# facebookresearch/actionmesh

Hardware: NVIDIA H100
Metric: denoiser_steps_per_sec (higher is better)
Workload: dtype bf16

## Files before the change

### actionmesh_b200/csrc/gemm.cu

```cuda
#include <atomic>
#include <cstdlib>
#include "common.cuh"
#include "ptx.cuh"
#include "../../include/actionmesh_b200.h"

namespace amb {

constexpr int BM = 128;
constexpr int BK = 64;
constexpr int GEMM_THREADS = 384;
constexpr int CLUSTER = 2;
constexpr int GROUP_M = 8;
constexpr int EPI_BATCH = 4;

struct GemmParams {
  int M, N, K;
  int k_split_blocks;
  void* C;
  long long ldc;
  int c_fp32;
  const float* bias;
  const void* residual;
  long long ldr;
  int res_fp32;
  int act;
  const float* col_scale;
  int grp_rows, grp_stride, row_off;
  int norm_cols, norm_seg;
  const float* norm_w0;
  const float* norm_w1;
  float norm_eps;
  int rope_cols;
  const float* rope_cos;
  const float* rope_sin;
  int rope_rows_per_pos;
  void* C2;
  long long ldc2;
};

__device__ __forceinline__ float gelu_erf(float x) {
  const float ax = fabsf(x);
  float t;
  asm("rcp.approx.ftz.f32 %0, %1;" : "=f"(t) : "f"(fmaf(0.3275911f * 0.70710678118654752440f, ax, 1.0f)));
  float p = fmaf(t, 1.061405429f, -1.453152027f);
  p = fmaf(p, t, 1.421413741f);
  p = fmaf(p, t, -0.284496736f);
  p = fmaf(p, t, 0.254829592f);
  const float e = ex2_approx(ax * ax * (-0.5f * 1.4426950408889634f));
  const float q = 0.5f * (p * t) * e;
  return x * (x >= 0.0f ? 1.0f - q : q);
}

template <int BN>
struct GemmSmem {
  static constexpr int STAGES = BN == 128 ? 6 : 8;
  static constexpr int A_BYTES = BM * BK * 2;
  static constexpr int B_BYTES = BN * BK * 2;
  static constexpr int STAGE_BYTES = A_BYTES + B_BYTES;
  static constexpr int BAR_OFFSET = STAGES * STAGE_BYTES;
  static constexpr int TOTAL = BAR_OFFSET + 2 * STAGES * 8 + 1024;
};

__device__ __forceinline__ void store2(void* C, int c_fp32, long long off, float v0, float v1) {
  if (c_fp32) *reinterpret_cast<float2*>(reinterpret_cast<float*>(C) + off) = make_float2(v0, v1);
  else *reinterpret_cast<uint32_t*>(reinterpret_cast<__nv_bfloat16*>(C) + off) = pack_bf16(v0, v1);
}
__device__ __forceinline__ float2 load2(const void* R, int r_fp32, long long off) {
  if (r_fp32) return *reinterpret_cast<const float2*>(reinterpret_cast<const float*>(R) + off);
  return unpack_bf16(*reinterpret_cast<const uint32_t*>(reinterpret_cast<const __nv_bfloat16*>(R) + off));
}

__device__ __forceinline__ void finish_pair(const GemmParams& p, float v0, float v1, float2 r, long long drow, int col,
                                            bool valid) {
  if (p.bias) {
    const float2 b = __ldg(reinterpret_cast<const float2*>(p.bias + col));
    v0 += b.x; v1 += b.y;
  }
  if (p.act == 1) {
    v0 = gelu_erf(v0);
    v1 = gelu_erf(v1);
  }
  if (p.col_scale) {
    const float2 s = __ldg(reinterpret_cast<const float2*>(p.col_scale + col));
    v0 *= s.x; v1 *= s.y;
  }
  if (!valid) return;
  if (p.residual) { v0 += r.x; v1 += r.y; }
  store2(p.C, p.c_fp32, drow * p.ldc + col, v0, v1);
  if (p.C2) store2(p.C2, 0, drow * p.ldc2 + col, v0, v1);
}

template <int BN>
__device__ __forceinline__ void epilogue_tile(const GemmParams& p, const float* acc, int n0, int r0) {
  const int q = threadIdx.x & 3;
  long long drow[2];
  bool valid[2];
  int row[2] = {r0, r0 + 8};
#pragma unroll
  for (int h = 0; h < 2; ++h) {
    valid[h] = row[h] < p.M;
    drow[h] = row[h];
    if (p.grp_rows > 0) drow[h] = (long long)(row[h] / p.grp_rows) * p.grp_stride + (row[h] % p.grp_rows) + p.row_off;
  }
  if constexpr (BN == 128) {
    const bool do_norm = n0 < p.norm_cols, do_rope = n0 < p.rope_cols;
    if (do_norm || do_rope) {
      float rs[2] = {1.0f, 1.0f};
      float2 nw[16];
      if (do_norm) {
        const float* w = (n0 < p.norm_seg) ? p.norm_w0 : p.norm_w1;
#pragma unroll
        for (int i = 0; i < 16; ++i) nw[i] = __ldg(reinterpret_cast<const float2*>(w + 8 * i + 2 * q));
        float ss0 = 0.f, ss1 = 0.f;
#pragma unroll
        for (int i = 0; i < 16; ++i) {
          ss0 += acc[4 * i] * acc[4 * i] + acc[4 * i + 1] * acc[4 * i + 1];
          ss1 += acc[4 * i + 2] * acc[4 * i + 2] + acc[4 * i + 3] * acc[4 * i + 3];
        }
        ss0 += __shfl_xor_sync(0xffffffffu, ss0, 1);
        ss1 += __shfl_xor_sync(0xffffffffu, ss1, 1);
        ss0 += __shfl_xor_sync(0xffffffffu, ss0, 2);
        ss1 += __shfl_xor_sync(0xffffffffu, ss1, 2);
        rs[0] = rsqrtf(ss0 * (1.0f / 128.0f) + p.norm_eps);
        rs[1] = rsqrtf(ss1 * (1.0f / 128.0f) + p.norm_eps);
      }
#pragma unroll
      for (int h = 0; h < 2; ++h) {
        float rc[16], rsn[16];
        if (do_rope) {
          const int pos = (valid[h] ? row[h] : 0) / p.rope_rows_per_pos;
          const float* cs = p.rope_cos + (long long)pos * 64;
          const float* sn = p.rope_sin + (long long)pos * 64;
#pragma unroll
          for (int i = 0; i < 16; ++i) {
            rc[i] = __ldg(cs + 4 * i + q);
            rsn[i] = __ldg(sn + 4 * i + q);
          }
        }
#pragma unroll
        for (int i = 0; i < 16; ++i) {
          const int lc = 8 * i + 2 * q;
          float v0 = acc[4 * i + 2 * h], v1 = acc[4 * i + 2 * h + 1];
          if (do_norm) {
            v0 *= rs[h] * nw[i].x;
            v1 *= rs[h] * nw[i].y;
          }
          if (do_rope) {
            const float c = rc[i], s = rsn[i];
            const float x = v0, y = v1;
            v0 = x * c - y * s;
            v1 = y * c + x * s;
          }
          if (valid[h]) store2(p.C, p.c_fp32, drow[h] * p.ldc + n0 + lc, v0, v1);
        }
      }
      return;
    }
  }
#pragma unroll
  for (int i0 = 0; i0 < BN / 8; i0 += EPI_BATCH) {
    float2 r[EPI_BATCH][2];
#pragma unroll
    for (int i = 0; i < EPI_BATCH; ++i)
#pragma unroll
      for (int h = 0; h < 2; ++h)
        r[i][h] = (p.residual && valid[h]) ? load2(p.residual, p.res_fp32, drow[h] * p.ldr + n0 + 8 * (i0 + i) + 2 * q)
                                           : make_float2(0.f, 0.f);
#pragma unroll
    for (int i = 0; i < EPI_BATCH; ++i) {
      const int col = n0 + 8 * (i0 + i) + 2 * q;
      const float* a = acc + 4 * (i0 + i);
      finish_pair(p, a[0], a[1], r[i][0], drow[0], col, valid[0]);
      finish_pair(p, a[2], a[3], r[i][1], drow[1], col, valid[1]);
    }
  }
}

template <int BN>
__device__ __forceinline__ void wgmma_tile_k16(float* acc, uint64_t adesc, uint64_t bdesc) {
  if constexpr (BN == 128) wgmma_ss_n128(acc, adesc, bdesc, 1u);
  else wgmma_ss_n64(acc, adesc, bdesc, 1u);
}

__device__ __forceinline__ void unit_tile(int u, int num_mp, int num_n, uint32_t rank, int& m0, int& nt) {
  const int band = u / (GROUP_M * num_n);
  const int first = band * GROUP_M;
  const int rows = min(GROUP_M, num_mp - first);
  const int r = u - band * GROUP_M * num_n;
  m0 = ((first + r % rows) * CLUSTER + (int)rank) * BM;
  nt = r / rows;
}

template <int BN>
__global__ void __cluster_dims__(CLUSTER, 1, 1) __launch_bounds__(GEMM_THREADS, 1)
gemm_bf16_kernel(const __grid_constant__ CUtensorMap tmA, const __grid_constant__ CUtensorMap tmA2,
                 const __grid_constant__ CUtensorMap tmB, const GemmParams p) {
  using L = GemmSmem<BN>;
  constexpr int STAGES = L::STAGES;
  constexpr int B_HALF = L::B_BYTES / CLUSTER;
  extern __shared__ uint8_t smem_raw[];
  uint8_t* smem = reinterpret_cast<uint8_t*>((reinterpret_cast<uintptr_t>(smem_raw) + 1023) & ~uintptr_t(1023));
  uint64_t* full_bar = reinterpret_cast<uint64_t*>(smem + L::BAR_OFFSET);
  uint64_t* empty_bar = full_bar + STAGES;

  const int wg = __shfl_sync(0xffffffffu, threadIdx.x >> 7, 0);
  const int warp = threadIdx.x >> 5;
  const int lane = threadIdx.x & 31;
  const uint32_t rank = cluster_ctarank();
  if (threadIdx.x == 0) {
    tma_prefetch_desc(&tmA);
    tma_prefetch_desc(&tmA2);
    tma_prefetch_desc(&tmB);
    for (int s = 0; s < STAGES; ++s) {
      mbar_init(&full_bar[s], 1);
      mbar_init(&empty_bar[s], 4 * CLUSTER);
    }
    fence_mbar_init();
  }
  cluster_sync();

  const int num_n = p.N / BN;
  const int num_mp = (p.M + CLUSTER * BM - 1) / (CLUSTER * BM);
  const int num_units = num_mp * num_n;
  const int cluster = blockIdx.x / CLUSTER, num_clusters = gridDim.x / CLUSTER;
  const int num_kb = p.K / BK;

  if (wg == 0) {
    reg_dealloc<40>();
    if (warp == 0) {
      int s = 0;
      uint32_t phase = 0;
      for (int u = cluster; u < num_units; u += num_clusters) {
        int m0, nt;
        unit_tile(u, num_mp, num_n, rank, m0, nt);
        const int n0 = nt * BN;
        for (int kb = 0; kb < num_kb; ++kb) {
          mbar_wait(&empty_bar[s], phase ^ 1);
          if (elect_one()) {
            mbar_expect_tx(&full_bar[s], L::STAGE_BYTES);
            uint8_t* sa = smem + s * L::STAGE_BYTES;
            uint8_t* sb = sa + L::A_BYTES;
            if (kb < p.k_split_blocks) tma_load_2d(sa, &tmA, &full_bar[s], kb * BK, m0, kEvictNormal);
            else tma_load_2d(sa, &tmA2, &full_bar[s], (kb - p.k_split_blocks) * BK, m0, kEvictNormal);
            tma_load_2d_multicast(sb + rank * B_HALF, &tmB, &full_bar[s], kb * BK, n0 + (int)rank * (BN / CLUSTER),
                                  (uint16_t)((1u << CLUSTER) - 1), kEvictLast);
          }
          __syncwarp();
          if (++s == STAGES) { s = 0; phase ^= 1; }
        }
      }
      for (int j = 0; j < STAGES; ++j) {
        mbar_wait(&empty_bar[s], phase ^ 1);
        if (++s == STAGES) { s = 0; phase ^= 1; }
      }
    }
  } else {
    reg_alloc<232>();
    const uint32_t my_turn = wg, other_turn = 3 - wg;
    const int n_local = (num_units - cluster + num_clusters - 1) / num_clusters;
    for (int i = wg - 1; i < n_local; i += 2) {
      int m0, nt;
      unit_tile(cluster + i * num_clusters, num_mp, num_n, rank, m0, nt);
      const int n0 = nt * BN;
      float acc[2][BN / 2];
#pragma unroll
      for (int h = 0; h < 2; ++h)
#pragma unroll
        for (int j = 0; j < BN / 2; ++j) acc[h][j] = 0.f;
      const long long g0 = (long long)i * num_kb;
      int s = (int)(g0 % STAGES), s_prev = s;
      uint32_t phase = (uint32_t)((g0 / STAGES) & 1);
      if (i > 0) named_bar_sync(my_turn, 256);
      for (int kb = 0; kb < num_kb; ++kb) {
        mbar_wait_watched(&full_bar[s], phase);
        const uint32_t a_addr = smem_u32(smem + s * L::STAGE_BYTES);
        const uint64_t adesc0 = make_desc_kmajor_sw128(a_addr);
        const uint64_t adesc1 = make_desc_kmajor_sw128(a_addr + 64 * 128);
        const uint64_t bdesc = make_desc_kmajor_sw128(a_addr + L::A_BYTES);
        wgmma_fence();
#pragma unroll
        for (int k = 0; k < BK / 16; ++k) {
          wgmma_tile_k16<BN>(acc[0], adesc0 + 2 * k, bdesc + 2 * k);
          wgmma_tile_k16<BN>(acc[1], adesc1 + 2 * k, bdesc + 2 * k);
        }
        wgmma_commit();
        wgmma_wait<1>();
        if (kb > 0) {
          __syncwarp();
          if (lane < CLUSTER) mbar_arrive_cluster(&empty_bar[s_prev], lane);
        }
        s_prev = s;
        if (++s == STAGES) { s = 0; phase ^= 1; }
      }
      if (i + 1 < n_local) named_bar_arrive(other_turn, 256);
      wgmma_wait<0>();
#pragma unroll
      for (int h = 0; h < 2; ++h)
#pragma unroll
        for (int j = 0; j < BN / 2; ++j) reg_fence(acc[h][j]);
      __syncwarp();
      if (lane < CLUSTER) mbar_arrive_cluster(&empty_bar[s_prev], lane);
      if (m0 < p.M) {
        const int r0 = m0 + (warp & 3) * 16 + (lane >> 2);
        epilogue_tile<BN>(p, acc[0], n0, r0);
        epilogue_tile<BN>(p, acc[1], n0, r0 + 64);
      }
    }
  }
  __syncwarp();
  cluster_sync();
}

static GemmParams make_params(const amb_gemm_args* a) {
  GemmParams p;
  p.M = a->m; p.N = a->n; p.K = a->k;
  p.k_split_blocks = a->a2 ? a->k_split / BK : 0x7fffffff;
  p.C = a->c; p.ldc = a->ldc; p.c_fp32 = a->c_fp32;
  p.bias = a->bias;
  p.residual = a->residual; p.ldr = a->ldr; p.res_fp32 = a->res_fp32;
  p.act = a->act;
  p.col_scale = a->col_scale;
  p.grp_rows = a->grp_rows; p.grp_stride = a->grp_stride; p.row_off = a->row_off;
  p.norm_cols = a->norm_cols; p.norm_seg = a->norm_seg;
  p.norm_w0 = a->norm_w0; p.norm_w1 = a->norm_w1 ? a->norm_w1 : a->norm_w0;
  p.norm_eps = a->norm_eps;
  p.rope_cols = a->rope_cols; p.rope_cos = a->rope_cos; p.rope_sin = a->rope_sin;
  p.rope_rows_per_pos = a->rope_rows_per_pos > 0 ? a->rope_rows_per_pos : 1;
  p.C2 = a->c2; p.ldc2 = a->ldc2;
  return p;
}

template <int BN>
static int max_active_clusters(int* out) {
  static std::atomic<int> cached[16];
  int dev = 0;
  AMB_CHECK_CUDA(cudaGetDevice(&dev));
  if (dev < 16 && cached[dev].load() > 0) {
    *out = cached[dev].load();
    return AMB_OK;
  }
  cudaLaunchConfig_t cfg = {};
  cfg.gridDim = dim3(CLUSTER * num_sms(), 1, 1);
  cfg.blockDim = dim3(GEMM_THREADS, 1, 1);
  cfg.dynamicSmemBytes = GemmSmem<BN>::TOTAL;
  int n = 0;
  AMB_CHECK_CUDA(cudaOccupancyMaxActiveClusters(&n, gemm_bf16_kernel<BN>, &cfg));
  AMB_CHECK_ARG(n > 0, "gemm: no %d-CTA cluster of %d B shared memory fits on device %d", CLUSTER, GemmSmem<BN>::TOTAL, dev);
  if (dev < 16) cached[dev].store(n);
  *out = n;
  return AMB_OK;
}

template <int BN>
static int launch_gemm(const amb_gemm_args* a, cudaStream_t stream) {
  using L = GemmSmem<BN>;
  CUtensorMap tmA, tmA2, tmB;
  const int k1 = (a->a2 != nullptr) ? a->k_split : a->k;
  {
    uint64_t dims[2] = {(uint64_t)k1, (uint64_t)a->m};
    uint64_t str[1] = {(uint64_t)a->lda * 2};
    uint32_t box[2] = {BK, BM};
    int r = encode_tmap_bf16(&tmA, a->a, 2, dims, str, box);
    if (r) return r;
  }
  if (a->a2) {
    uint64_t dims[2] = {(uint64_t)(a->k - a->k_split), (uint64_t)a->m};
    uint64_t str[1] = {(uint64_t)a->lda2 * 2};
    uint32_t box[2] = {BK, BM};
    int r = encode_tmap_bf16(&tmA2, a->a2, 2, dims, str, box);
    if (r) return r;
  } else {
    tmA2 = tmA;
  }
  {
    uint64_t dims[2] = {(uint64_t)a->k, (uint64_t)a->n};
    uint64_t str[1] = {(uint64_t)a->ldw * 2};
    uint32_t box[2] = {BK, BN / CLUSTER};
    int r = encode_tmap_bf16(&tmB, a->w, 2, dims, str, box);
    if (r) return r;
  }
  GemmParams p = make_params(a);
  auto kern = gemm_bf16_kernel<BN>;
  {
    int r = ensure_smem_optin(kern, L::TOTAL);
    if (r) return r;
  }
  int clusters = 0;
  {
    int r = max_active_clusters<BN>(&clusters);
    if (r) return r;
  }
  const long long num_mp = ((long long)a->m + CLUSTER * BM - 1) / (CLUSTER * BM);
  const long long num_units = (long long)(a->n / BN) * num_mp;
  AMB_CHECK_ARG(num_units < 0x7fffffffLL, "gemm: too many tiles (m=%d n=%d)", a->m, a->n);
  const unsigned grid = (unsigned)(CLUSTER * (num_units < clusters ? num_units : clusters));
  kern<<<grid, GEMM_THREADS, L::TOTAL, stream>>>(tmA, tmA2, tmB, p);
  AMB_CHECK_CUDA(cudaGetLastError());
  return AMB_OK;
}

}

using namespace amb;

extern "C" int amb_gemm_bf16(const amb_gemm_args* a, amb_stream_t stream) {
  AMB_CHECK_ARG(a && a->a && a->w && a->c, "gemm: null pointer");
  AMB_CHECK_ARG(a->m > 0 && a->n > 0 && a->k > 0, "gemm: bad shape m=%d n=%d k=%d", a->m, a->n, a->k);
  AMB_CHECK_ARG(a->k % BK == 0, "gemm: k=%d must be a multiple of %d", a->k, BK);
  AMB_CHECK_ARG(a->n % 64 == 0, "gemm: n=%d must be a multiple of 64", a->n);
  AMB_CHECK_ARG(a->lda % 8 == 0 && a->ldw % 8 == 0 && a->ldc % 8 == 0, "gemm: lda/ldw/ldc must be multiples of 8 elements");
  AMB_CHECK_ARG(!a->a2 || (a->k_split > 0 && a->k_split < a->k && a->k_split % BK == 0 && a->lda2 % 8 == 0),
                "gemm: bad k_split %d", a->k_split);
  AMB_CHECK_ARG(!a->residual || a->ldr % 8 == 0, "gemm: ldr must be a multiple of 8");
  AMB_CHECK_ARG(a->act == 0 || a->act == 1, "gemm: unknown activation %d", a->act);
  AMB_CHECK_ARG(!a->c2 || a->ldc2 % 8 == 0, "gemm: ldc2 must be a multiple of 8");
  if (a->norm_cols > 0 || a->rope_cols > 0) {
    AMB_CHECK_ARG(a->n % 128 == 0 && a->norm_cols % 128 == 0 && a->rope_cols % 128 == 0,
                  "gemm: head epilogue needs n, norm_cols, rope_cols multiples of 128");
    AMB_CHECK_ARG(a->norm_cols == 0 || (a->norm_w0 && a->norm_seg % 128 == 0), "gemm: norm weights / norm_seg (multiple of 128) required");
    AMB_CHECK_ARG(a->rope_cols == 0 || (a->rope_cos && a->rope_sin), "gemm: rope tables required");
    AMB_CHECK_ARG(!a->residual && a->act == 0 && !a->col_scale && !a->c2, "gemm: head epilogue excludes residual/activation/col_scale/c2");
  }
  cudaStream_t s = (cudaStream_t)stream;
  if (a->n % 128 == 0) return launch_gemm<128>(a, s);
  return launch_gemm<64>(a, s);
}
```

Before: 1.033.

## Add 2x2 cluster GEMM variant multicasting both A and B tiles

Generalizes the GEMM cluster to a CM x CN grid, so a 4-CTA cluster shares A tiles across the N direction as well as B tiles across the M direction via TMA multicast. This cuts L2/HBM traffic per output tile for large-N GEMMs. A heuristic compares wave counts for the 2- and 4-CTA configs, biased toward 4 when K is large, and an env var can override it. The cost is coarser scheduling units (256x256), which can worsen wave quantization and load balance, plus extra occupancy queries at launch.

```diff
diff --git a/actionmesh_b200/csrc/gemm.cu b/actionmesh_b200/csrc/gemm.cu
--- a/actionmesh_b200/csrc/gemm.cu
+++ b/actionmesh_b200/csrc/gemm.cu
@@ -9,7 +9,7 @@
 constexpr int BM = 128;
 constexpr int BK = 64;
 constexpr int GEMM_THREADS = 384;
-constexpr int CLUSTER = 2;
+constexpr int CM = 2;
 constexpr int GROUP_M = 8;
 constexpr int EPI_BATCH = 4;
 
@@ -182,22 +182,25 @@
   else wgmma_ss_n64(acc, adesc, bdesc, 1u);
 }
 
-__device__ __forceinline__ void unit_tile(int u, int num_mp, int num_n, uint32_t rank, int& m0, int& nt) {
-  const int band = u / (GROUP_M * num_n);
+template <int CN>
+__device__ __forceinline__ void unit_tile(int u, int num_mp, int num_np, int rm, int rn, int& m0, int& nt) {
+  const int band = u / (GROUP_M * num_np);
   const int first = band * GROUP_M;
   const int rows = min(GROUP_M, num_mp - first);
-  const int r = u - band * GROUP_M * num_n;
-  m0 = ((first + r % rows) * CLUSTER + (int)rank) * BM;
-  nt = r / rows;
-}
-
-template <int BN>
-__global__ void __cluster_dims__(CLUSTER, 1, 1) __launch_bounds__(GEMM_THREADS, 1)
+  const int r = u - band * GROUP_M * num_np;
+  m0 = ((first + r % rows) * CM + rm) * BM;
+  nt = (r / rows) * CN + rn;
+}
+
+template <int BN, int CN>
+__global__ void __cluster_dims__(CM * CN, 1, 1) __launch_bounds__(GEMM_THREADS, 1)
 gemm_bf16_kernel(const __grid_constant__ CUtensorMap tmA, const __grid_constant__ CUtensorMap tmA2,
                  const __grid_constant__ CUtensorMap tmB, const GemmParams p) {
   using L = GemmSmem<BN>;
   constexpr int STAGES = L::STAGES;
-  constexpr int B_HALF = L::B_BYTES / CLUSTER;
+  constexpr int CLUSTER = CM * CN;
+  constexpr int B_PART = L::B_BYTES / CM;
+  constexpr int A_PART = L::A_BYTES / CN;
   extern __shared__ uint8_t smem_raw[];
   uint8_t* smem = reinterpret_cast<uint8_t*>((reinterpret_cast<uintptr_t>(smem_raw) + 1023) & ~uintptr_t(1023));
   uint64_t* full_bar = reinterpret_cast<uint64_t*>(smem + L::BAR_OFFSET);
@@ -219,9 +222,10 @@
   }
   cluster_sync();
 
-  const int num_n = p.N / BN;
-  const int num_mp = (p.M + CLUSTER * BM - 1) / (CLUSTER * BM);
-  const int num_units = num_mp * num_n;
+  const int rm = (int)(rank % CM), rn = (int)(rank / CM);
+  const int num_np = p.N / (BN * CN);
+  const int num_mp = (p.M + CM * BM - 1) / (CM * BM);
+  const int num_units = num_mp * num_np;
   const int cluster = blockIdx.x / CLUSTER, num_clusters = gridDim.x / CLUSTER;
   const int num_kb = p.K / BK;
 
@@ -232,7 +236,7 @@
       uint32_t phase = 0;
       for (int u = cluster; u < num_units; u += num_clusters) {
         int m0, nt;
-        unit_tile(u, num_mp, num_n, rank, m0, nt);
+        unit_tile<CN>(u, num_mp, num_np, rm, rn, m0, nt);
         const int n0 = nt * BN;
         for (int kb = 0; kb < num_kb; ++kb) {
           mbar_wait(&empty_bar[s], phase ^ 1);
@@ -240,10 +244,16 @@
             mbar_expect_tx(&full_bar[s], L::STAGE_BYTES);
             uint8_t* sa = smem + s * L::STAGE_BYTES;
             uint8_t* sb = sa + L::A_BYTES;
-            if (kb < p.k_split_blocks) tma_load_2d(sa, &tmA, &full_bar[s], kb * BK, m0, kEvictNormal);
-            else tma_load_2d(sa, &tmA2, &full_bar[s], (kb - p.k_split_blocks) * BK, m0, kEvictNormal);
-            tma_load_2d_multicast(sb + rank * B_HALF, &tmB, &full_bar[s], kb * BK, n0 + (int)rank * (BN / CLUSTER),
-                                  (uint16_t)((1u << CLUSTER) - 1), kEvictLast);
+            const CUtensorMap* ta = kb < p.k_split_blocks ? &tmA : &tmA2;
+            const int ka = (kb < p.k_split_blocks ? kb : kb - p.k_split_blocks) * BK;
+            if constexpr (CN == 1) {
+              tma_load_2d(sa, ta, &full_bar[s], ka, m0, kEvictNormal);
+            } else {
+              tma_load_2d_multicast(sa + rn * A_PART, ta, &full_bar[s], ka, m0 + rn * (BM / CN),
+                                    (uint16_t)(((1u << CM * (CN - 1)) | 1u) << rm), kEvictNormal);
+            }
+            tma_load_2d_multicast(sb + rm * B_PART, &tmB, &full_bar[s], kb * BK, n0 + rm * (BN / CM),
+                                  (uint16_t)(((1u << CM) - 1) << (CM * rn)), kEvictLast);
           }
           __syncwarp();
           if (++s == STAGES) { s = 0; phase ^= 1; }
@@ -260,7 +270,7 @@
     const int n_local = (num_units - cluster + num_clusters - 1) / num_clusters;
     for (int i = wg - 1; i < n_local; i += 2) {
       int m0, nt;
-      unit_tile(cluster + i * num_clusters, num_mp, num_n, rank, m0, nt);
+      unit_tile<CN>(cluster + i * num_clusters, num_mp, num_np, rm, rn, m0, nt);
       const int n0 = nt * BN;
       float acc[2][BN / 2];
 #pragma unroll
@@ -330,9 +340,14 @@
   return p;
 }
 
-template <int BN>
+template <int BN, int CN>
 static int max_active_clusters(int* out) {
+  constexpr int CLUSTER = CM * CN;
   static std::atomic<int> cached[16];
+  {
+    int r = ensure_smem_optin(gemm_bf16_kernel<BN, CN>, GemmSmem<BN>::TOTAL);
+    if (r) return r;
+  }
   int dev = 0;
   AMB_CHECK_CUDA(cudaGetDevice(&dev));
   if (dev < 16 && cached[dev].load() > 0) {
@@ -344,29 +359,35 @@
   cfg.blockDim = dim3(GEMM_THREADS, 1, 1);
   cfg.dynamicSmemBytes = GemmSmem<BN>::TOTAL;
   int n = 0;
-  AMB_CHECK_CUDA(cudaOccupancyMaxActiveClusters(&n, gemm_bf16_kernel<BN>, &cfg));
+  AMB_CHECK_CUDA(cudaOccupancyMaxActiveClusters(&n, gemm_bf16_kernel<BN, CN>, &cfg));
   AMB_CHECK_ARG(n > 0, "gemm: no %d-CTA cluster of %d B shared memory fits on device %d", CLUSTER, GemmSmem<BN>::TOTAL, dev);
   if (dev < 16) cached[dev].store(n);
   *out = n;
   return AMB_OK;
 }
 
-template <int BN>
+template <int BN, int CN>
+static long long gemm_units(const amb_gemm_args* a) {
+  return (long long)(a->n / (BN * CN)) * (((long long)a->m + CM * BM - 1) / (CM * BM));
+}
+
+template <int BN, int CN>
 static int launch_gemm(const amb_gemm_args* a, cudaStream_t stream) {
   using L = GemmSmem<BN>;
+  constexpr int CLUSTER = CM * CN;
   CUtensorMap tmA, tmA2, tmB;
   const int k1 = (a->a2 != nullptr) ? a->k_split : a->k;
   {
     uint64_t dims[2] = {(uint64_t)k1, (uint64_t)a->m};
     uint64_t str[1] = {(uint64_t)a->lda * 2};
-    uint32_t box[2] = {BK, BM};
+    uint32_t box[2] = {BK, BM / CN};
     int r = encode_tmap_bf16(&tmA, a->a, 2, dims, str, box);
     if (r) return r;
   }
   if (a->a2) {
     uint64_t dims[2] = {(uint64_t)(a->k - a->k_split), (uint64_t)a->m};
     uint64_t str[1] = {(uint64_t)a->lda2 * 2};
-    uint32_t box[2] = {BK, BM};
+    uint32_t box[2] = {BK, BM / CN};
     int r = encode_tmap_bf16(&tmA2, a->a2, 2, dims, str, box);
     if (r) return r;
   } else {
@@ -375,23 +396,18 @@
   {
     uint64_t dims[2] = {(uint64_t)a->k, (uint64_t)a->n};
     uint64_t str[1] = {(uint64_t)a->ldw * 2};
-    uint32_t box[2] = {BK, BN / CLUSTER};
+    uint32_t box[2] = {BK, BN / CM};
     int r = encode_tmap_bf16(&tmB, a->w, 2, dims, str, box);
     if (r) return r;
   }
   GemmParams p = make_params(a);
-  auto kern = gemm_bf16_kernel<BN>;
-  {
-    int r = ensure_smem_optin(kern, L::TOTAL);
-    if (r) return r;
-  }
+  auto kern = gemm_bf16_kernel<BN, CN>;
   int clusters = 0;
   {
-    int r = max_active_clusters<BN>(&clusters);
-    if (r) return r;
-  }
-  const long long num_mp = ((long long)a->m + CLUSTER * BM - 1) / (CLUSTER * BM);
-  const long long num_units = (long long)(a->n / BN) * num_mp;
+    int r = max_active_clusters<BN, CN>(&clusters);
+    if (r) return r;
+  }
+  const long long num_units = gemm_units<BN, CN>(a);
   AMB_CHECK_ARG(num_units < 0x7fffffffLL, "gemm: too many tiles (m=%d n=%d)", a->m, a->n);
   const unsigned grid = (unsigned)(CLUSTER * (num_units < clusters ? num_units : clusters));
   kern<<<grid, GEMM_THREADS, L::TOTAL, stream>>>(tmA, tmA2, tmB, p);
@@ -422,6 +438,22 @@
     AMB_CHECK_ARG(!a->residual && a->act == 0 && !a->col_scale && !a->c2, "gemm: head epilogue excludes residual/activation/col_scale/c2");
   }
   cudaStream_t s = (cudaStream_t)stream;
-  if (a->n % 128 == 0) return launch_gemm<128>(a, s);
-  return launch_gemm<64>(a, s);
-}
+  if (a->n % 128 != 0) return launch_gemm<64, 1>(a, s);
+  if (a->n % 256 != 0) return launch_gemm<128, 1>(a, s);
+  const char* force = getenv("AMB_GEMM_CLUSTER");
+  bool quad;
+  if (force && force[0] == '2' && !force[1]) {
+    quad = false;
+  } else if (force && force[0] == '4' && !force[1]) {
+    quad = true;
+  } else {
+    AMB_CHECK_ARG(!force || !force[0], "gemm: AMB_GEMM_CLUSTER=%s (expected 2 or 4)", force);
+    int c2 = 0, c4 = 0;
+    int r = max_active_clusters<128, 1>(&c2);
+    if (!r) r = max_active_clusters<128, 2>(&c4);
+    if (r) return r;
+    const long long t2 = (gemm_units<128, 1>(a) + c2 - 1) / c2, t4 = (gemm_units<128, 2>(a) + c4 - 1) / c4;
+    quad = 100 * t4 <= (a->k >= 4096 ? 125 : 110) * t2;
+  }
+  return quad ? launch_gemm<128, 2>(a, s) : launch_gemm<128, 1>(a, s);
+}
```

New measurement: 1.063, median of 6. +2.9%, better.
